# nlesc-dirac/sagecal

Measured on NVIDIA H100. Metric: baseline_visibilities_per_sec_predict_jacobian, higher is better.
Workload: dtype f64

## Files before the change

### sagecal_b200/csrc/internal.cuh

```cuda
#pragma once
#include <cuda_runtime.h>
#include <stdint.h>
#include <stdio.h>
#include <stdlib.h>

#define DB_CHECK(call)                                                                          \
  do {                                                                                          \
    cudaError_t err__ = (call);                                                                 \
    if (err__ != cudaSuccess) {                                                                 \
      fprintf(stderr, "dirac_b200: CUDA error %s at %s:%d: %s\n", cudaGetErrorName(err__),      \
              __FILE__, __LINE__, cudaGetErrorString(err__));                                   \
      exit(1);          \
    }                                                                                           \
  } while (0)


#define TILE_P 8
#define TILE_Q 32
#define TILE_THREADS (TILE_P * TILE_Q)

struct TileDesc {
  short pb, qb;
};

// ... 229 lines not shown

struct GramArgs {
  const double2 *coh;
  const unsigned char *flag;
  const TileDesc *tiles;
  double *T;
  long long R;
  int N, Nbase;
  int k0;
  int t_begin, t_end, t_step;
};

struct AssembleArgs {
  const double *T;
  const double *pblk;
  double *JTJ;
  double *Hst;
  const TileDesc *tiles;
  const short2 *blpq;
  int N, Nbase;
};

struct BatchAssembleArgs {
  const double *T;
  const double *pp;
  const int *list;
  const int *tix;
  const int *poff;
  double *JTJ;
  double *Hst;
  const TileDesc *tiles;
  const short2 *blpq;
  int N, Nbase;
};

enum { DB_OPT_CP_ROWS = 0, DB_OPT_LINE_DIRECT = 1, DB_OPT_OS_CONSISTENT = 2,
       DB_OPT_RTR_NU_UNJOINED = 3, DB_OPT_ADMM_LM = 4, DB_OPT_COUNT = 8 };
int db_opt(int id);
int db_sm_count();
static inline int db_cp_max_slices(int Nbase, int tilesz) {
  const int nbg = (Nbase + 255) / 256;
  int nsl = (db_sm_count() + nbg - 1) / nbg;
  if ((tilesz + 31) / 32 > nsl) nsl = (tilesz + 31) / 32;
  return nsl;
}

extern "C" {
void db_launch_coh_to_planar(const double2 *src, double2 *dst, long long r0, int nr, int M,
                             long long R, cudaStream_t st);
void db_launch_coh_from_planar(const double2 *src, double2 *dst, long long r0, int nr, int M,
                               long long R, cudaStream_t st);
void db_launch_vis_to_planar(const double2 *src, double2 *dst, long long R, cudaStream_t st);
void db_launch_vis_from_planar(const double2 *src, double2 *dst, long long R, cudaStream_t st);
void db_launch_grad_tma(const GradArgs *a, int ntile, cudaStream_t st);
void db_launch_grad_window_tma(const GradArgs *a, int ntile, long long r_lo, long long r_hi,
                               cudaStream_t st);
void db_launch_grad_band_tma(const GradArgs *a, int ntile, int nchan, cudaStream_t st);
int db_cluster_pass_nblocks(int ntile, int nt, int tslice);
void db_launch_cluster_pass(const ClusterPassArgs *a, int ntile, cudaStream_t st);
int db_cluster_pass_forms_hidden(int N, int Nbase);
void db_launch_coh_gram(const GramArgs *a, int ntile, int nk, cudaStream_t st);
void db_launch_assemble(const AssembleArgs *a, int ntile, cudaStream_t st);
void db_launch_copy_add_diag(const double *A0, double *A, int n, double mu, cudaStream_t st);
int db_chol_max_n();
int db_chol_available();
size_t db_chol_ws_doubles(int n);
int db_tri_available(int n);
void db_chol_set_step(const double *pcur, double *pnew, double *sc, double *zero);
void db_launch_tri_solve(const double *L, int n, const double *b, double *x, cudaStream_t st);
void db_launch_tri_solve_ld(const double *L, int ld, int n, const double *b, double *x,
                            cudaStream_t st);
void db_launch_chol_factor_batched(const double *A, int n, const double *mu, double *ws,
                                   long long ws_stride, int *info, int nb, cudaStream_t st);
void db_launch_chol_solve(const double *A, int n, double mu, const double *b, double *x, double *ws,
                          int *info, cudaStream_t st);
int db_bigtri_available(int n);
size_t db_bigtri_ws_doubles(int n);
// ... 13 lines not shown
```

### sagecal_b200/csrc/kernels_lm.cu

```cuda
#include "internal.cuh"

struct Gram {
  double d[4];
  double2 o[6];
  __device__ __forceinline__ double2 at(int u, int v) const {
    if (u == v) return make_double2(d[u], 0.0);
    int lo = u < v ? u : v, hi = u < v ? v : u;
    int idx = (lo == 0) ? (hi - 1) : (lo == 1 ? (hi + 1) : 5);
    double2 z = o[idx];
    return (u < v) ? z : make_double2(z.x, -z.y);
  }
};


__device__ __forceinline__ void assemble_baseline(const AssembleArgs &a, int p, int q, long long b,
                                                  int sub) {
  Gram G;
  {
    const double2 *Tb = reinterpret_cast<const double2 *>(a.T + b * 16);
    double2 t0 = Tb[0], t1 = Tb[1];
    G.d[0] = t0.x; G.d[1] = t0.y; G.d[2] = t1.x; G.d[3] = t1.y;
#pragma unroll
    for (int z = 0; z < 6; z++) G.o[z] = Tb[2 + z];
  }
  double2 Jp[4], Jq[4];
  load_jones(a.pblk, p, Jp);
  load_jones(a.pblk, q, Jq);
  const int ld = 8 * a.N;
#pragma unroll
  for (int i = 0; i < 2; i++)
#pragma unroll
    for (int l = 0; l < 2; l++)
#pragma unroll
      for (int j = 0; j < 2; j++)
#pragma unroll
        for (int lp = 0; lp < 2; lp++) {
          double2 z = make_double2(0.0, 0.0);
#pragma unroll
          for (int aa = 0; aa < 2; aa++)
#pragma unroll
            for (int bb = 0; bb < 2; bb++) {
              double2 jj = cmul(Jq[2 * j + aa], Jp[2 * i + bb]);
              cfma(z, jj, G.at(2 * l + aa, 2 * bb + lp));
            }
          if (sub != ((i * 2 + l) * 2 + j) * 2 + lp) continue;
          const int r0 = 8 * p + 2 * (2 * i + l);
          const int c0 = 8 * q + 2 * (2 * j + lp);
          a.JTJ[(long long)r0 * ld + c0] = z.x;
          a.JTJ[(long long)r0 * ld + c0 + 1] = z.y;
          a.JTJ[(long long)(r0 + 1) * ld + c0] = z.y;
          a.JTJ[(long long)(r0 + 1) * ld + c0 + 1] = -z.x;
          a.JTJ[(long long)c0 * ld + r0] = z.x;
          a.JTJ[(long long)(c0 + 1) * ld + r0] = z.y;
          a.JTJ[(long long)c0 * ld + r0 + 1] = z.y;
          a.JTJ[(long long)(c0 + 1) * ld + r0 + 1] = -z.x;
        }
  double2 Qq[4], Qp[4];
  mat_ahb(Jq, Jq, Qq);
  mat_ahb(Jp, Jp, Qp);
  double2 Hp[4], Hq[4];
#pragma unroll
  for (int l = 0; l < 2; l++)
#pragma unroll
    for (int lp = 0; lp < 2; lp++) {
      double2 hp = make_double2(0.0, 0.0), hq = make_double2(0.0, 0.0);
#pragma unroll
      for (int aa = 0; aa < 2; aa++)
#pragma unroll
        for (int bb = 0; bb < 2; bb++) {
          cfma(hp, Qq[2 * aa + bb], G.at(2 * lp + bb, 2 * l + aa));
          cfma(hq, Qp[2 * aa + bb], G.at(2 * aa + l, 2 * bb + lp));
        }
      Hp[2 * l + lp] = hp;
      Hq[2 * l + lp] = hq;
    }
  if (sub == 0) atomicAdd(a.Hst + 4 * p + 0, Hp[0].x);
  if (sub == 1) atomicAdd(a.Hst + 4 * p + 1, Hp[3].x);
  if (sub == 2) atomicAdd(a.Hst + 4 * p + 2, Hp[1].x);
  if (sub == 3) atomicAdd(a.Hst + 4 * p + 3, Hp[1].y);
  if (sub == 4) atomicAdd(a.Hst + 4 * q + 0, Hq[0].x);
  if (sub == 5) atomicAdd(a.Hst + 4 * q + 1, Hq[3].x);
  if (sub == 6) atomicAdd(a.Hst + 4 * q + 2, Hq[1].x);
  if (sub == 7) atomicAdd(a.Hst + 4 * q + 3, Hq[1].y);
}

__device__ __forceinline__ void assemble_lin(const AssembleArgs &a) {
  const long long gid = (long long)blockIdx.x * blockDim.x + threadIdx.x;
  const long long b = gid >> 4;
  if (b >= a.Nbase) return;
  const short2 pq = a.blpq[b];
  assemble_baseline(a, pq.x, pq.y, b, (int)(gid & 15));
}

__global__ void __launch_bounds__(256)
k_assemble_offdiag(AssembleArgs a) {
  assemble_lin(a);
}

__global__ void __launch_bounds__(256)
k_assemble_offdiag_batched(BatchAssembleArgs b) {
  const int k = b.list[blockIdx.y];
  AssembleArgs a;
  a.T = b.T + (long long)b.tix[k] * b.Nbase * 16;
  a.pblk = b.pp + b.poff[k];
  a.JTJ = b.JTJ + (long long)blockIdx.y * 64 * b.N * b.N;
  a.Hst = b.Hst + (long long)blockIdx.y * 4 * b.N;
  a.tiles = b.tiles;
  a.blpq = b.blpq;
  a.N = b.N;
  a.Nbase = b.Nbase;
  assemble_lin(a);
}

__device__ __forceinline__ void assemble_diag_station(const double *__restrict__ Hst,
                                                      double *__restrict__ JTJ, int N, int s);

__global__ void k_assemble_diag(const double *__restrict__ Hst, double *__restrict__ JTJ, int N) {
  int s = blockIdx.x * blockDim.x + threadIdx.x;
  if (s >= N) return;
  assemble_diag_station(Hst, JTJ, N, s);
}
__global__ void k_assemble_diag_batched(const double *__restrict__ Hst, double *__restrict__ JTJ,
                                        int N) {
  int s = blockIdx.x * blockDim.x + threadIdx.x;
  if (s >= N) return;
  assemble_diag_station(Hst + (long long)blockIdx.y * 4 * N, JTJ + (long long)blockIdx.y * 64 * N * N,
                        N, s);
}
__device__ __forceinline__ void assemble_diag_station(const double *__restrict__ Hst,
                                                      double *__restrict__ JTJ, int N, int s) {
  const double h00 = Hst[4 * s], h11 = Hst[4 * s + 1], hr = Hst[4 * s + 2], hi = Hst[4 * s + 3];
  const int ld = 8 * N;
  for (int i = 0; i < 2; i++) {
    double blk[4][4] = {{h00, 0.0, hr, hi}, {0.0, h00, -hi, hr}, {hr, -hi, h11, 0.0},
                        {hi, hr, 0.0, h11}};
    for (int r = 0; r < 8; r++)
      for (int c = 0; c < 8; c++) {
        double v = 0.0;
        if ((r >> 2) == i && (c >> 2) == i) v = blk[r & 3][c & 3];
        if ((r >> 2) == i) JTJ[(long long)(8 * s + r) * ld + 8 * s + c] = v;
      }
  }
}

__global__ void __launch_bounds__(128)
k_batch_mu0(const double *__restrict__ Hst, double *__restrict__ mu, int N, double tau) {
  __shared__ double sv[4];
  const double *H = Hst + (long long)blockIdx.x * 4 * N;
  double mx = 0.0;
  for (int s = threadIdx.x; s < N; s += blockDim.x) {
    const double a = H[4 * s], b = H[4 * s + 1];
    if (fabs(a) > fabs(mx)) mx = a;
    if (fabs(b) > fabs(mx)) mx = b;
  }
#pragma unroll
  for (int o = 16; o > 0; o >>= 1) {
    const double other = __shfl_xor_sync(0xffffffffu, mx, o);
    if (fabs(other) > fabs(mx)) mx = other;
  }
  if ((threadIdx.x & 31) == 0) sv[threadIdx.x >> 5] = mx;
  __syncthreads();
  if (threadIdx.x == 0) {
    for (int i = 1; i < 4; i++)
      if (fabs(sv[i]) > fabs(mx)) mx = sv[i];
    mu[blockIdx.x] = tau * mx;
  }
}

__global__ void k_batch_add_diag(const double *__restrict__ A0, double *__restrict__ A,
                                 const double *__restrict__ mu, int n) {
  const long long nn = (long long)n * n;
  const long long i = (long long)blockIdx.x * blockDim.x + threadIdx.x;
  if (i < nn) {
    double v = A0[(long long)blockIdx.y * nn + i];
    if (i / n == i % n) v += mu[blockIdx.y];
    A[(long long)blockIdx.y * nn + i] = v;
  }
}

__global__ void k_copy_add_diag(const double *__restrict__ A0, double *__restrict__ A, int n,
                                double mu) {
  long long i = (long long)blockIdx.x * blockDim.x + threadIdx.x;
  long long nn = (long long)n * n;
  if (i < nn) {
    double v = A0[i];
    if (i / n == i % n) v += mu;
    A[i] = v;
  }
}

__global__ void k_extract_diag(const double *__restrict__ A, double *__restrict__ dst, int n) {
// ... 39 lines not shown
  if (i < n) g[i] = g[i] - 0.5 * y[i] - 0.5 * rho * (p[i] - bz[i]);
}

extern "C" {
void db_launch_lm_aug_rhs(double *jte, const double *p, const double *y, const double *bz,
                          double rho, int n, cudaStream_t st) {
  k_lm_aug_rhs<<<(n + 255) / 256, 256, 0, st>>>(jte, p, y, bz, rho, n);
}
void db_launch_lm_step(const double *p, const double *Dp, const double *jte, double *pnew,
                       double *sc, double *zero, int n, cudaStream_t st) {
  k_lm_step<<<1, 512, 0, st>>>(p, Dp, jte, pnew, sc, zero, n);
}
void db_launch_extract_diag(const double *A, double *dst, int n, cudaStream_t st) {
  k_extract_diag<<<(n + 127) / 128, 128, 0, st>>>(A, dst, n);
}
void db_launch_assemble(const AssembleArgs *a, int ntile, cudaStream_t st) {
  (void)ntile;
  k_assemble_offdiag<<<(a->Nbase * 16 + 255) / 256, 256, 0, st>>>(*a);
  k_assemble_diag<<<(a->N + 63) / 64, 64, 0, st>>>(a->Hst, a->JTJ, a->N);
}
void db_launch_assemble_batched(const BatchAssembleArgs *b, int ntile, int nb, double tau,
                                double *mu, double *Afac, cudaStream_t st) {
  (void)ntile;
  dim3 g1((b->Nbase * 16 + 255) / 256, nb);
  k_assemble_offdiag_batched<<<g1, 256, 0, st>>>(*b);
  dim3 g2((b->N + 63) / 64, nb);
  k_assemble_diag_batched<<<g2, 64, 0, st>>>(b->Hst, b->JTJ, b->N);
  k_batch_mu0<<<nb, 128, 0, st>>>(b->Hst, mu, b->N, tau);
  if (!Afac) return;
  const int n = 8 * b->N;
  const long long nn = (long long)n * n;
  dim3 g3((unsigned)((nn + 255) / 256), nb);
  k_batch_add_diag<<<g3, 256, 0, st>>>(b->JTJ, Afac, mu, n);
}
void db_launch_copy_add_diag(const double *A0, double *A, int n, double mu, cudaStream_t st) {
  long long nn = (long long)n * n;
  k_copy_add_diag<<<(unsigned)((nn + 255) / 256), 256, 0, st>>>(A0, A, n, mu);
}
}
```

### sagecal_b200/csrc/lm.cu

```cuda
#include <float.h>
#include <math.h>
#include <string.h>
#include <vector>

#include "../../include/dirac_b200.h"
#include "problem.h"

#define CS_CHECK(call)                                                                     \
  do {                                                                                     \
    cusolverStatus_t s__ = (call);                                                         \
    if (s__ != CUSOLVER_STATUS_SUCCESS) {                                                  \
      fprintf(stderr, "dirac_b200: cuSOLVER error %d at %s:%d\n", (int)s__, __FILE__, __LINE__); \
      exit(1);                                                                             \
    }                                                                                      \
  } while (0)
#define CB_CHECK(call)                                                                     \
  do {                                                                                     \
    cublasStatus_t s__ = (call);                                                           \
    if (s__ != CUBLAS_STATUS_SUCCESS) {                                                    \
      fprintf(stderr, "dirac_b200: cuBLAS error %d at %s:%d\n", (int)s__, __FILE__, __LINE__); \
      exit(1);                                                                             \
    }                                                                                      \
  } while (0)

extern "C" {
void db_launch_weighted_jtj(const WeightedJtjArgs *a, int ntile, cudaStream_t st);
void db_launch_sum_abs(const double2 *v, long long R, long long r0, long long r1, double *partials,
                       double *out, unsigned int *counter, cudaStream_t st);
void db_launch_update_weights(const double2 *e, double2 *wt, long long R, long long r0,
                              long long r1, double nu0, double *partials, double *out,
                              unsigned int *counter, cudaStream_t st);
void db_launch_scale_vis(double2 *v, long long R, long long r0, long long r1, double alpha,
                         int set_const, cudaStream_t st);
void db_launch_extract_diag(const double *A, double *dst, int n, cudaStream_t st);
void db_launch_assemble_batched(const BatchAssembleArgs *b, int ntile, int nb, double tau,
                                double *mu, double *Afac, cudaStream_t st);
void db_launch_lm_step(const double *p, const double *Dp, const double *jte, double *pnew,
                       double *sc, double *zero, int n, cudaStream_t st);
void db_launch_os_shift(const double2 *e, const double2 *wt, double2 *eps, double2 *wout, long long R,
                        long long row_sub0, long long nrow_sub, long long row_chunk0, long long kl,
                        long long nJ, cudaStream_t st);
}

template <typename T>
static T *dalloc(size_t n) {
  return (T *)db_malloc(n * sizeof(T) + 16);
}

void db_lm_init(dirac_b200_problem *pr) {
  LMWork &w = pr->lm;
  if (w.ready) return;
// ... 7 lines not shown
  w.JTJ = dalloc<double>((size_t)n8 * n8);
  w.JTe = d.scal + 64 + n8;
  w.JTe_new = d.scal + 64 + 2 * n8;
  w.Hst = dalloc<double>((size_t)4 * d.N);
  w.Dp = d.scal + 64;
  w.pnew = dalloc<double>(n8);
  w.plast = dalloc<double>(n8);
  w.pold = dalloc<double>(n8);
  w.devinfo = reinterpret_cast<int *>(d.scal + 64 + 3 * n8);
  w.tau = dalloc<double>(n8);
  w.svdS = w.svdU = w.svdVT = nullptr;
  w.wbuf = w.ebuf = nullptr;
  w.os_eps = w.os_w = nullptr;
  w.HP = w.HQ = nullptr;
  w.JB = w.LB = nullptr;
  w.pref_slot = (int *)malloc(sizeof(int) * d.M);
  for (int k = 0; k < d.M; k++) w.pref_slot[k] = -1;
  w.jtj0_cur = nullptr;
  w.jtj_spec = nullptr;
  {
    const int nbg = (d.Nbase + 255) / 256;
    const int nsl = db_cp_max_slices(d.Nbase, d.tilesz);
    w.jte_part = dalloc<double>((size_t)nbg * (nsl + 1) * n8);
  }
  DB_CHECK(cudaEventCreateWithFlags(&w.ev_mail, cudaEventDisableTiming));
  DB_CHECK(cudaMallocHost((void **)&w.h_vec, sizeof(double) * (5 * n8 + 4 * d.N + 64)));
  static cusolverDnHandle_t g_cs = nullptr;
  static cublasHandle_t g_cb = nullptr;
  if (!g_cs) {
    CS_CHECK(cusolverDnCreate(&g_cs));
// ... 43 lines not shown
  if (w.os_eps) return;
  w.os_eps = dalloc<double2>((size_t)4 * pr->d.R);
  w.os_w = dalloc<double2>((size_t)4 * pr->d.R);
}

void db_lm_free(dirac_b200_problem *pr) {
  LMWork &w = pr->lm;
  if (!w.ready) return;
  db_free(w.T); db_free(w.Tsub); db_free(w.JTJ0); db_free(w.JTJ);
  db_free(w.Hst); db_free(w.pnew); db_free(w.plast); db_free(w.pold); db_free(w.jte_part);
  db_free(w.tau); db_free(w.cswork); db_free(w.dbuf);
  if (w.bt_ws) db_free(w.bt_ws);
  if (w.svdS) { db_free(w.svdS); db_free(w.svdU); db_free(w.svdVT); }
  if (w.wbuf) { db_free(w.wbuf); db_free(w.ebuf); db_free(w.HP); db_free(w.HQ); }
  if (w.os_eps) { db_free(w.os_eps); db_free(w.os_w); }
  if (w.JB) {
    db_free(w.JB); db_free(w.LB); db_free(w.HB); db_free(w.mu_dev); db_free(w.binfo_dev);
    db_free(w.LBptr_dev); db_free(w.blist_dev); db_free(w.btix_dev); db_free(w.bpoff_dev);
    cudaFreeHost(w.h_mu); cudaFreeHost(w.h_binfo);
  }
  free(w.pref_slot);
  cudaEventDestroy(w.ev_mail);
  cudaFreeHost(w.h_vec);
  free(w.T_valid);
  w.ready = false;
}

static int pick_tslice(const DevProblem &d, int nt) {
  int target_ctas = db_sm_count();
  int slices = (target_ctas + d.ntile - 1) / d.ntile;
  if (slices < 1) slices = 1;
  int ts = (nt + slices - 1) / slices;
// ... 39 lines not shown
  db_count_launch(1);
}

static void gram(dirac_b200_problem *pr, int k, int t0, int t1, int step, double *Tdst) {
  DevProblem &d = pr->d;
  GramArgs a;
  a.coh = d.coh; a.flag = d.flag; a.tiles = d.tiles; a.T = Tdst; a.R = d.R; a.N = d.N;
  a.Nbase = d.Nbase; a.k0 = k; a.t_begin = t0; a.t_end = t1; a.t_step = step;
  db_prof_begin(3, (double)((t1 - t0 + step - 1) / step) * d.Nbase * 65.0 + 128.0 * d.Nbase,
                d.stream);
  db_launch_coh_gram(&a, d.ntile, 1, d.stream);
  db_prof_end(d.stream);
  db_count_launch(1);
}

static void assemble(dirac_b200_problem *pr, const double *T, const double *pblk_dev,
                     double *JTJ) {
  DevProblem &d = pr->d;
  LMWork &w = pr->lm;
  DB_CHECK(cudaMemsetAsync(w.Hst, 0, sizeof(double) * 4 * d.N, d.stream));
  AssembleArgs a;
  a.T = T; a.pblk = pblk_dev; a.JTJ = JTJ; a.Hst = w.Hst; a.tiles = d.tiles; a.blpq = d.blpq;
  a.N = d.N;
  a.Nbase = d.Nbase;
  db_prof_begin(4, 128.0 * d.Nbase + 8.0 * 64.0 * d.N * d.N, d.stream);
  db_launch_assemble(&a, d.ntile, d.stream);
  db_prof_end(d.stream);
  db_count_launch(2);
}

static void weighted_jtj(dirac_b200_problem *pr, int k, int t0, int t1, const double *pblk_dev,
                         const double2 *wt, double *JTJ) {
  DevProblem &d = pr->d;
  LMWork &w = pr->lm;
  const int n = w.n8;
  DB_CHECK(cudaMemsetAsync(JTJ, 0, sizeof(double) * (size_t)n * n, d.stream));
  DB_CHECK(cudaMemsetAsync(w.HP, 0, sizeof(double) * 20 * d.N, d.stream));
  DB_CHECK(cudaMemsetAsync(w.HQ, 0, sizeof(double) * 20 * d.N, d.stream));
  if (t1 <= t0) return;
  WeightedJtjArgs a;
  a.coh_k = d.coh + (size_t)k * 4 * d.R;
  a.wt = wt; a.flag = d.flag; a.pblk = pblk_dev; a.tiles = d.tiles; a.JTJ = JTJ; a.HP = w.HP;
  a.HQ = w.HQ; a.R = d.R; a.N = d.N; a.Nbase = d.Nbase; a.t_begin = t0; a.t_end = t1;
// ... 22 lines not shown
static int enqueue_solve(dirac_b200_problem *pr, double mu, int linsolv, double eps1) {
  DevProblem &d = pr->d;
  LMWork &w = pr->lm;
  const int n = w.n8;
  int *hinfo = (int *)(w.h_vec + 4 * n + 4 * d.N);
  hinfo[0] = hinfo[1] = 0;
  if (linsolv == 0 && w.own_chol) {
    db_prof_begin(5, 0.0, d.stream);
    db_launch_chol_solve(w.jtj0_cur ? w.jtj0_cur : w.JTJ0, n, mu, w.JTe, w.Dp, w.cswork, w.devinfo,
                         d.stream);
    db_prof_end(d.stream);
    db_count_launch(1);
    w.step_fused = w.step_armed;
    return 1;
  }
  db_launch_copy_add_diag(w.jtj0_cur ? w.jtj0_cur : w.JTJ0, w.JTJ, n, mu, d.stream);
  db_count_launch(1);
  DB_CHECK(cudaMemcpyAsync(w.Dp, w.JTe, sizeof(double) * n, cudaMemcpyDeviceToDevice, d.stream));
  db_prof_begin(5, 0.0, d.stream);
  if (linsolv == 0) {
    CS_CHECK(cusolverDnDpotrf(w.cs, CUBLAS_FILL_MODE_LOWER, n, w.JTJ, n, w.cswork, w.lwork,
                              w.devinfo));
    if (w.bt_ws) {
      DB_CHECK(cudaMemsetAsync(w.devinfo + 1, 0, sizeof(int), d.stream));
      db_launch_bigtri_solve(w.JTJ, n, n, w.JTe, w.Dp, w.bt_ws, ++w.bt_epoch, 1, d.stream);
      db_count_launch(4);
    } else {
      CS_CHECK(cusolverDnDpotrs(w.cs, CUBLAS_FILL_MODE_LOWER, n, 1, w.JTJ, n, w.Dp, n,
                                w.devinfo + 1));
      db_count_launch(2);
    }
  } else if (linsolv == 1) {
// ... 37 lines not shown
  return 1;
}

static double nrm2sq(const double *v, int n) {
  double s = 0.0;
  for (int i = 0; i < n; i++) s += v[i] * v[i];
  return s;
}

void db_prefactor_sweep(dirac_b200_problem *pr, double tau) {
  DevProblem &d = pr->d;
  db_lm_init(pr);
  LMWork &w = pr->lm;
  const int n = w.n8;
  const size_t nn = (size_t)n * n;
  if ((double)d.M * nn * 16.0 > 24e9) return;
  const bool own_batch = w.own_chol && db_tri_available(n) && !getenv("DIRAC_B200_BATCH_CUSOLVER");
  const size_t lstride = own_batch ? db_chol_ws_doubles(n) : nn;
  w.lb_stride = lstride;
  w.lb_ld = own_batch ? 32 * ((n + 31) / 32) : n;
  if (!w.JB) {
    w.JB = dalloc<double>(nn * d.M);
    w.LB = dalloc<double>(lstride * d.M);
    w.HB = dalloc<double>((size_t)4 * d.N * d.M);
    w.mu_dev = dalloc<double>(d.M);
    w.binfo_dev = dalloc<int>(2 * d.M);
    w.LBptr_dev = (double **)dalloc<double *>(d.M);
    w.blist_dev = dalloc<int>(d.M);
    w.btix_dev = dalloc<int>(d.M);
    w.bpoff_dev = dalloc<int>(d.M);
    DB_CHECK(cudaMallocHost((void **)&w.h_mu, sizeof(double) * d.M));
    DB_CHECK(cudaMallocHost((void **)&w.h_binfo, sizeof(int) * 2 * d.M));
    std::vector<int> tix(d.M), poff(d.M);
    std::vector<double *> ptr(d.M);
    for (int k = 0; k < d.M; k++) {
      tix[k] = d.h_clus[k].chunk0;
      poff[k] = d.h_chunk_poff[d.h_clus[k].chunk0];
// ... 24 lines not shown
    db_prof_end(d.stream);
    db_count_launch(1);
    for (int kk = k; kk < k1; kk++) w.T_valid[d.h_clus[kk].chunk0] = 1;
    k = k1;
  }
  for (int k = 0; k < d.M; k++) {
    w.pref_slot[k] = -1;
    if (d.h_clus[k].nchunk != 1) continue;
    w.pref_slot[k] = (int)list.size();
    list.push_back(k);
  }
  const int nb = (int)list.size();
  if (nb == 0) return;
  DB_CHECK(cudaMemcpyAsync(w.blist_dev, list.data(), sizeof(int) * nb, cudaMemcpyHostToDevice,
                           d.stream));
  DB_CHECK(cudaMemsetAsync(w.HB, 0, sizeof(double) * 4 * d.N * nb, d.stream));
  BatchAssembleArgs b;
  b.T = w.T; b.pp = d.pp; b.list = w.blist_dev; b.tix = w.btix_dev; b.poff = w.bpoff_dev;
  b.JTJ = w.JB; b.Hst = w.HB; b.tiles = d.tiles; b.blpq = d.blpq; b.N = d.N; b.Nbase = d.Nbase;
  db_prof_begin(4, nb * (128.0 * d.Nbase + 8.0 * 64.0 * d.N * d.N), d.stream);
  db_launch_assemble_batched(&b, d.ntile, nb, tau, w.mu_dev, own_batch ? nullptr : w.LB, d.stream);
  db_prof_end(d.stream);
  db_count_launch(4);
  db_prof_begin(5, 0.0, d.stream);
  if (own_batch) {
    db_launch_chol_factor_batched(w.JB, n, w.mu_dev, w.LB, (long long)lstride, w.binfo_dev, nb,
                                  d.stream);
    db_count_launch(1);
  } else if (n <= 1024) {
    CS_CHECK(cusolverDnDpotrfBatched(w.cs, CUBLAS_FILL_MODE_LOWER, n, w.LBptr_dev, n, w.binfo_dev, nb));
    db_count_launch(1);
  } else {
    enum { NS = 4 };
    static cudaStream_t fs[NS];
    static cusolverDnHandle_t fh[NS];
    static double *fwork[NS];
    static int flwork = 0;
    static cudaEvent_t fev[NS], fstart;
// ... 230 lines not shown
      break;
    }
    if (os && randomize) {
      subI.resize(Nsubsets);
      for (int i = 0; i < Nsubsets; ++i) {
        const int j = rand() % (i + 1);
        subI[i] = subI[j];
        subI[j] = i;
      }
    }
    for (int ositer = 0; ositer < max_os_iter; ositer++) {
      double mx = 0.0;
      const int slot = (!wt && !os && kiter == 0 && linsolv == 0) ? w.pref_slot[k] : -1;
      const bool prefac = slot >= 0;
      const bool need_mx = (kiter == 0) && !prefac;
      w.jtj0_cur = prefac ? w.JB + (size_t)slot * n * n : nullptr;
      if (os) {
        const int l = randomize ? subI[ositer] : (os_shift + kiter + ositer) % Nsubsets;
        os_subset_system(pr, k, t0, t1, l, pblk_dev, wt);
        DB_CHECK(cudaMemcpyAsync(hjte, w.JTe, sizeof(double) * n, cudaMemcpyDeviceToHost,
                                 d.stream));
      } else if (prefac) {
        w.pref_slot[k] = -1;
      } else if (wt) {
        weighted_jtj(pr, k, t0, t1, pblk_dev, wt, w.JTJ0);
      } else if (w.jtj_spec) {
        w.jtj0_cur = w.jtj_spec;
        w.jtj_spec = nullptr;
      } else {
        assemble(pr, Tfull, pblk_dev, w.JTJ0);
      }
      if (need_mx) {
        if (wt || os_misaligned) {
          db_launch_extract_diag(w.JTJ0, w.JTe_new, n, d.stream);
          db_count_launch(1);
          DB_CHECK(cudaMemcpyAsync(hsc, w.JTe_new, sizeof(double) * n, cudaMemcpyDeviceToHost,
                                   d.stream));
        } else {
          DB_CHECK(cudaMemcpyAsync(hH, w.Hst, sizeof(double) * 4 * d.N, cudaMemcpyDeviceToHost,
                                   d.stream));
        }
      }
      if (need_mx || os) db_stream_sync(d.stream);
      if (need_mx) {
        if (wt || os_misaligned) {
// ... 410 lines not shown
  int t0, t1;
  chunk_range(d, clus, chunk, &t0, &t1);
  db_upload_vis(pr, xd, w.dbuf);
  db_upload_vis(pr, wt, w.wbuf);
  DB_CHECK(cudaMemcpyAsync(w.pnew, pblk, sizeof(double) * n, cudaMemcpyHostToDevice, d.stream));
  db_cluster_pass(pr, clus, w.pnew, w.dbuf, nullptr, 1, 0, w.JTe, 1, t0, t1, w.wbuf);
  weighted_jtj(pr, clus, t0, t1, w.pnew, w.wbuf, w.JTJ0);
  double c = db_read_scalar(pr, 1);
  if (JTe) DB_CHECK(cudaMemcpy(JTe, w.JTe, sizeof(double) * n, cudaMemcpyDeviceToHost));
  if (JTJ)
    DB_CHECK(cudaMemcpy(JTJ, w.JTJ0, sizeof(double) * (size_t)n * n, cudaMemcpyDeviceToHost));
  DB_CHECK(cudaGetLastError());
  return c;
}

extern "C" void dirac_b200_os_normal_eq(dirac_b200_problem *pr, int clus, int chunk, int l,
                                        const double *pblk, const double *xd, const double *wt,
                                        double *JTJ, double *JTe, long long *path) {
  DevProblem &d = pr->d;
  db_lm_init(pr);
  robust_init(pr);
  LMWork &w = pr->lm;
  const int n = w.n8;
  int t0, t1;
  chunk_range(d, clus, chunk, &t0, &t1);
  db_upload_vis(pr, xd, w.dbuf);
  if (wt) db_upload_vis(pr, wt, w.wbuf);
  DB_CHECK(cudaMemcpyAsync(w.pnew, pblk, sizeof(double) * n, cudaMemcpyHostToDevice, d.stream));
  const OsPath p = os_subset_system(pr, clus, t0, t1, l, w.pnew, wt ? w.wbuf : nullptr);
  DB_CHECK(cudaMemcpyAsync(JTe, w.JTe, sizeof(double) * n, cudaMemcpyDeviceToHost, d.stream));
// ... 110 lines not shown
```

### sagecal_b200/csrc/problem.h

```cpp
#pragma once
#include <cusolverDn.h>
#include <cublas_v2.h>

#include <vector>

#include "../../include/dirac_b200.h"
#include "internal.cuh"

struct LMWork {
  bool ready;
  int n8;
  double *T;
  unsigned char *T_valid;
  double *Tsub;
  double *JTJ0, *JTJ;
  double *JTe, *JTe_new;
  double *Hst;
  double *Dp;
  double *pnew;
  double *h_vec;
  int *devinfo;
  double *cswork;
  int lwork;
  bool own_chol;
// ... 13 lines not shown
  double2 *os_eps, *os_w;
  double *HP, *HQ;
  double *plast;
  double *pold;
  double *JB, *LB;
  size_t lb_stride;
  int lb_ld, binfo_step;
  double *HB;
  double *mu_dev;
  double *h_mu;
  int *binfo_dev, *h_binfo;
  double **LBptr_dev;
  int *blist_dev, *btix_dev, *bpoff_dev;
  int *pref_slot;
  const double *jtj0_cur;
};

struct dirac_b200_problem {
  DevProblem d;
  double *partials;
  int npartials;
  double2 *res;
  double2 *vis_stage;
  double *g;
  LMWork lm;
  int own_stream;
  int rank, world;
  void (*allreduce)(void *dev, long long count, void *stream, void *user);
  void *comm_user;
  int m_global;
// ... 119 lines not shown
```

Measured before the change: 6.222 billion.

## Restructure LM normal-equation assembly into station-sum and tiled damped-assembly kernels

Replaces the per-baseline JTJ assembly, which used atomics for the station Hessian diagonals and a separate diagonal kernel, with two kernels. One computes per-station sums with warp reductions and no atomics. The other writes JTJ tiles with vectorized stores, adding the damping mu directly and optionally writing only the lower triangle. This removes the memset, the copy_add_diag pass and the batched add-diag pass, and can drop the JB buffer when it is not needed. The cost is recomputing the tiles for each damping trial when assembling in place. The measured workload is predict/jacobian visibilities, which may not exercise this LM path.

```diff
diff --git a/sagecal_b200/csrc/internal.cuh b/sagecal_b200/csrc/internal.cuh
--- a/sagecal_b200/csrc/internal.cuh
+++ b/sagecal_b200/csrc/internal.cuh
@@ -267,23 +267,15 @@
 struct AssembleArgs {
   const double *T;
   const double *pblk;
-  double *JTJ;
-  double *Hst;
-  const TileDesc *tiles;
-  const short2 *blpq;
-  int N, Nbase;
-};
-
-struct BatchAssembleArgs {
-  const double *T;
-  const double *pp;
   const int *list;
   const int *tix;
   const int *poff;
   double *JTJ;
+  long long stride;
   double *Hst;
-  const TileDesc *tiles;
-  const short2 *blpq;
+  const double *mu_dev;
+  double mu;
+  int lower;
   int N, Nbase;
 };
 
@@ -313,7 +305,9 @@
 void db_launch_cluster_pass(const ClusterPassArgs *a, int ntile, cudaStream_t st);
 int db_cluster_pass_forms_hidden(int N, int Nbase);
 void db_launch_coh_gram(const GramArgs *a, int ntile, int nk, cudaStream_t st);
-void db_launch_assemble(const AssembleArgs *a, int ntile, cudaStream_t st);
+void db_launch_station_sums(const AssembleArgs *a, int nb, cudaStream_t st);
+void db_launch_assemble_tiles(const AssembleArgs *a, int nb, cudaStream_t st);
+void db_launch_batch_mu0(const double *Hst, double *mu, int N, double tau, int nb, cudaStream_t st);
 void db_launch_copy_add_diag(const double *A0, double *A, int n, double mu, cudaStream_t st);
 int db_chol_max_n();
 int db_chol_available();
diff --git a/sagecal_b200/csrc/kernels_lm.cu b/sagecal_b200/csrc/kernels_lm.cu
--- a/sagecal_b200/csrc/kernels_lm.cu
+++ b/sagecal_b200/csrc/kernels_lm.cu
@@ -13,133 +13,144 @@
 };
 
 
-__device__ __forceinline__ void assemble_baseline(const AssembleArgs &a, int p, int q, long long b,
-                                                  int sub) {
+__device__ __forceinline__ long long pair_baseline(int p, int q, int N) {
+  return (long long)p * (2 * N - p - 1) / 2 + (q - p - 1);
+}
+
+__device__ __forceinline__ Gram load_gram(const double *T, long long b) {
   Gram G;
-  {
-    const double2 *Tb = reinterpret_cast<const double2 *>(a.T + b * 16);
-    double2 t0 = Tb[0], t1 = Tb[1];
-    G.d[0] = t0.x; G.d[1] = t0.y; G.d[2] = t1.x; G.d[3] = t1.y;
-#pragma unroll
-    for (int z = 0; z < 6; z++) G.o[z] = Tb[2 + z];
-  }
-  double2 Jp[4], Jq[4];
-  load_jones(a.pblk, p, Jp);
-  load_jones(a.pblk, q, Jq);
-  const int ld = 8 * a.N;
-#pragma unroll
-  for (int i = 0; i < 2; i++)
+  const double2 *Tb = reinterpret_cast<const double2 *>(T + b * 16);
+  const double2 t0 = __ldg(Tb), t1 = __ldg(Tb + 1);
+  G.d[0] = t0.x; G.d[1] = t0.y; G.d[2] = t1.x; G.d[3] = t1.y;
+#pragma unroll
+  for (int z = 0; z < 6; z++) G.o[z] = __ldg(Tb + 2 + z);
+  return G;
+}
+
+struct AsmSys {
+  const double *T, *J;
+  double *A, *H;
+  double mu;
+};
+__device__ __forceinline__ AsmSys asm_sys(const AssembleArgs &a, int y) {
+  AsmSys s;
+  if (a.list) {
+    const int k = a.list[y];
+    s.T = a.T + (long long)a.tix[k] * a.Nbase * 16;
+    s.J = a.pblk + a.poff[k];
+  } else {
+    s.T = a.T;
+    s.J = a.pblk;
+  }
+  s.A = a.JTJ + (long long)y * a.stride;
+  s.H = a.Hst + (long long)y * 4 * a.N;
+  s.mu = a.mu_dev ? a.mu_dev[y] : a.mu;
+  return s;
+}
+
+__global__ void __launch_bounds__(256)
+k_station_sums(AssembleArgs a) {
+  const AsmSys S = asm_sys(a, blockIdx.y);
+  const int s = blockIdx.x * 8 + (threadIdx.x >> 5);
+  const int lane = threadIdx.x & 31;
+  if (s >= a.N) return;
+  double h0 = 0.0, h1 = 0.0, h2 = 0.0, h3 = 0.0;
+  for (int o = lane; o < a.N; o += 32) {
+    if (o == s) continue;
+    const bool sp = s < o;
+    const Gram G = load_gram(S.T, sp ? pair_baseline(s, o, a.N) : pair_baseline(o, s, a.N));
+    double2 Jo[4], Qo[4];
+    load_jones(S.J, o, Jo);
+    mat_ahb(Jo, Jo, Qo);
+    double2 h[4];
 #pragma unroll
     for (int l = 0; l < 2; l++)
 #pragma unroll
-      for (int j = 0; j < 2; j++)
-#pragma unroll
-        for (int lp = 0; lp < 2; lp++) {
-          double2 z = make_double2(0.0, 0.0);
-#pragma unroll
-          for (int aa = 0; aa < 2; aa++)
-#pragma unroll
-            for (int bb = 0; bb < 2; bb++) {
-              double2 jj = cmul(Jq[2 * j + aa], Jp[2 * i + bb]);
-              cfma(z, jj, G.at(2 * l + aa, 2 * bb + lp));
-            }
-          if (sub != ((i * 2 + l) * 2 + j) * 2 + lp) continue;
-          const int r0 = 8 * p + 2 * (2 * i + l);
-          const int c0 = 8 * q + 2 * (2 * j + lp);
-          a.JTJ[(long long)r0 * ld + c0] = z.x;
-          a.JTJ[(long long)r0 * ld + c0 + 1] = z.y;
-          a.JTJ[(long long)(r0 + 1) * ld + c0] = z.y;
-          a.JTJ[(long long)(r0 + 1) * ld + c0 + 1] = -z.x;
-          a.JTJ[(long long)c0 * ld + r0] = z.x;
-          a.JTJ[(long long)(c0 + 1) * ld + r0] = z.y;
-          a.JTJ[(long long)c0 * ld + r0 + 1] = z.y;
-          a.JTJ[(long long)(c0 + 1) * ld + r0 + 1] = -z.x;
+      for (int lp = 0; lp < 2; lp++) {
+        double2 z = make_double2(0.0, 0.0);
+#pragma unroll
+        for (int aa = 0; aa < 2; aa++)
+#pragma unroll
+          for (int bb = 0; bb < 2; bb++)
+            cfma(z, Qo[2 * aa + bb], sp ? G.at(2 * lp + bb, 2 * l + aa) : G.at(2 * aa + l, 2 * bb + lp));
+        h[2 * l + lp] = z;
+      }
+    h0 += h[0].x;
+    h1 += h[3].x;
+    h2 += h[1].x;
+    h3 += h[1].y;
+  }
+  h0 = warp_sum(h0);
+  h1 = warp_sum(h1);
+  h2 = warp_sum(h2);
+  h3 = warp_sum(h3);
+  if (lane == 0) {
+    S.H[4 * s] = h0;
+    S.H[4 * s + 1] = h1;
+    S.H[4 * s + 2] = h2;
+    S.H[4 * s + 3] = h3;
+  }
+}
+
+__global__ void __launch_bounds__(256)
+k_assemble_tiles(AssembleArgs a) {
+  const int P = blockIdx.x;
+  const int qcta = blockIdx.y * 64;
+  if (a.lower && qcta + 64 <= P) return;
+  const int warp = threadIdx.x >> 5, lane = threadIdx.x & 31;
+  const int q0 = qcta + 8 * warp;
+  if (q0 >= a.N || (a.lower && q0 + 8 <= P)) return;
+  const AsmSys S = asm_sys(a, blockIdx.z);
+  const int Q = q0 + (lane >> 2);
+  const int jl = lane & 3, j = jl >> 1, lp = jl & 1;
+  const long long ld = 8ll * a.N;
+  if (Q == P) {
+    const double h00 = S.H[4 * P], h11 = S.H[4 * P + 1], hr = S.H[4 * P + 2], hi = S.H[4 * P + 3];
+    const double blk[4][4] = {{h00, 0.0, hr, hi}, {0.0, h00, -hi, hr}, {hr, -hi, h11, 0.0},
+                              {hi, hr, 0.0, h11}};
+#pragma unroll
+    for (int il = 0; il < 4; il++) {
+      const int i = il >> 1, l = il & 1;
+      double2 v0 = make_double2(0.0, 0.0), v1 = v0;
+      if (i == j) {
+        const double m = (l == lp) ? S.mu : 0.0;
+        v0 = lp ? make_double2(blk[2 * l][2], blk[2 * l][3]) : make_double2(blk[2 * l][0], blk[2 * l][1]);
+        v1 = lp ? make_double2(blk[2 * l + 1][2], blk[2 * l + 1][3])
+                : make_double2(blk[2 * l + 1][0], blk[2 * l + 1][1]);
+        v0.x += m;
+        v1.y += m;
+      }
+      const long long r0 = 8ll * P + 2 * il;
+      *reinterpret_cast<double2 *>(S.A + r0 * ld + 8ll * Q + 2 * jl) = v0;
+      *reinterpret_cast<double2 *>(S.A + (r0 + 1) * ld + 8ll * Q + 2 * jl) = v1;
+    }
+    return;
+  }
+  if (Q < a.N) {
+    const bool pq = P < Q;
+    const Gram G = load_gram(S.T, pq ? pair_baseline(P, Q, a.N) : pair_baseline(Q, P, a.N));
+    double2 JP[4], JQ[4];
+    load_jones(S.J, P, JP);
+    load_jones(S.J, Q, JQ);
+    const double2 Jj[2] = {j ? JQ[2] : JQ[0], j ? JQ[3] : JQ[1]};
+#pragma unroll
+    for (int il = 0; il < 4; il++) {
+      const int i = il >> 1, l = il & 1;
+      double2 z = make_double2(0.0, 0.0);
+#pragma unroll
+      for (int aa = 0; aa < 2; aa++)
+#pragma unroll
+        for (int bb = 0; bb < 2; bb++) {
+          if (pq)
+            cfma(z, cmul(Jj[aa], JP[2 * i + bb]),
+                 lp ? G.at(2 * l + aa, 2 * bb + 1) : G.at(2 * l + aa, 2 * bb));
+          else
+            cfma(z, cmul(JP[2 * i + aa], Jj[bb]), lp ? G.at(2 + aa, 2 * bb + l) : G.at(aa, 2 * bb + l));
         }
-  double2 Qq[4], Qp[4];
-  mat_ahb(Jq, Jq, Qq);
-  mat_ahb(Jp, Jp, Qp);
-  double2 Hp[4], Hq[4];
-#pragma unroll
-  for (int l = 0; l < 2; l++)
-#pragma unroll
-    for (int lp = 0; lp < 2; lp++) {
-      double2 hp = make_double2(0.0, 0.0), hq = make_double2(0.0, 0.0);
-#pragma unroll
-      for (int aa = 0; aa < 2; aa++)
-#pragma unroll
-        for (int bb = 0; bb < 2; bb++) {
-          cfma(hp, Qq[2 * aa + bb], G.at(2 * lp + bb, 2 * l + aa));
-          cfma(hq, Qp[2 * aa + bb], G.at(2 * aa + l, 2 * bb + lp));
-        }
-      Hp[2 * l + lp] = hp;
-      Hq[2 * l + lp] = hq;
+      const long long r0 = 8ll * P + 2 * il;
+      *reinterpret_cast<double2 *>(S.A + r0 * ld + 8ll * Q + 2 * jl) = z;
+      *reinterpret_cast<double2 *>(S.A + (r0 + 1) * ld + 8ll * Q + 2 * jl) = make_double2(z.y, -z.x);
     }
-  if (sub == 0) atomicAdd(a.Hst + 4 * p + 0, Hp[0].x);
-  if (sub == 1) atomicAdd(a.Hst + 4 * p + 1, Hp[3].x);
-  if (sub == 2) atomicAdd(a.Hst + 4 * p + 2, Hp[1].x);
-  if (sub == 3) atomicAdd(a.Hst + 4 * p + 3, Hp[1].y);
-  if (sub == 4) atomicAdd(a.Hst + 4 * q + 0, Hq[0].x);
-  if (sub == 5) atomicAdd(a.Hst + 4 * q + 1, Hq[3].x);
-  if (sub == 6) atomicAdd(a.Hst + 4 * q + 2, Hq[1].x);
-  if (sub == 7) atomicAdd(a.Hst + 4 * q + 3, Hq[1].y);
-}
-
-__device__ __forceinline__ void assemble_lin(const AssembleArgs &a) {
-  const long long gid = (long long)blockIdx.x * blockDim.x + threadIdx.x;
-  const long long b = gid >> 4;
-  if (b >= a.Nbase) return;
-  const short2 pq = a.blpq[b];
-  assemble_baseline(a, pq.x, pq.y, b, (int)(gid & 15));
-}
-
-__global__ void __launch_bounds__(256)
-k_assemble_offdiag(AssembleArgs a) {
-  assemble_lin(a);
-}
-
-__global__ void __launch_bounds__(256)
-k_assemble_offdiag_batched(BatchAssembleArgs b) {
-  const int k = b.list[blockIdx.y];
-  AssembleArgs a;
-  a.T = b.T + (long long)b.tix[k] * b.Nbase * 16;
-  a.pblk = b.pp + b.poff[k];
-  a.JTJ = b.JTJ + (long long)blockIdx.y * 64 * b.N * b.N;
-  a.Hst = b.Hst + (long long)blockIdx.y * 4 * b.N;
-  a.tiles = b.tiles;
-  a.blpq = b.blpq;
-  a.N = b.N;
-  a.Nbase = b.Nbase;
-  assemble_lin(a);
-}
-
-__device__ __forceinline__ void assemble_diag_station(const double *__restrict__ Hst,
-                                                      double *__restrict__ JTJ, int N, int s);
-
-__global__ void k_assemble_diag(const double *__restrict__ Hst, double *__restrict__ JTJ, int N) {
-  int s = blockIdx.x * blockDim.x + threadIdx.x;
-  if (s >= N) return;
-  assemble_diag_station(Hst, JTJ, N, s);
-}
-__global__ void k_assemble_diag_batched(const double *__restrict__ Hst, double *__restrict__ JTJ,
-                                        int N) {
-  int s = blockIdx.x * blockDim.x + threadIdx.x;
-  if (s >= N) return;
-  assemble_diag_station(Hst + (long long)blockIdx.y * 4 * N, JTJ + (long long)blockIdx.y * 64 * N * N,
-                        N, s);
-}
-__device__ __forceinline__ void assemble_diag_station(const double *__restrict__ Hst,
-                                                      double *__restrict__ JTJ, int N, int s) {
-  const double h00 = Hst[4 * s], h11 = Hst[4 * s + 1], hr = Hst[4 * s + 2], hi = Hst[4 * s + 3];
-  const int ld = 8 * N;
-  for (int i = 0; i < 2; i++) {
-    double blk[4][4] = {{h00, 0.0, hr, hi}, {0.0, h00, -hi, hr}, {hr, -hi, h11, 0.0},
-                        {hi, hr, 0.0, h11}};
-    for (int r = 0; r < 8; r++)
-      for (int c = 0; c < 8; c++) {
-        double v = 0.0;
-        if ((r >> 2) == i && (c >> 2) == i) v = blk[r & 3][c & 3];
-        if ((r >> 2) == i) JTJ[(long long)(8 * s + r) * ld + 8 * s + c] = v;
-      }
   }
 }
 
@@ -164,17 +175,6 @@
     for (int i = 1; i < 4; i++)
       if (fabs(sv[i]) > fabs(mx)) mx = sv[i];
     mu[blockIdx.x] = tau * mx;
-  }
-}
-
-__global__ void k_batch_add_diag(const double *__restrict__ A0, double *__restrict__ A,
-                                 const double *__restrict__ mu, int n) {
-  const long long nn = (long long)n * n;
-  const long long i = (long long)blockIdx.x * blockDim.x + threadIdx.x;
-  if (i < nn) {
-    double v = A0[(long long)blockIdx.y * nn + i];
-    if (i / n == i % n) v += mu[blockIdx.y];
-    A[(long long)blockIdx.y * nn + i] = v;
   }
 }
 
@@ -244,24 +244,14 @@
 void db_launch_extract_diag(const double *A, double *dst, int n, cudaStream_t st) {
   k_extract_diag<<<(n + 127) / 128, 128, 0, st>>>(A, dst, n);
 }
-void db_launch_assemble(const AssembleArgs *a, int ntile, cudaStream_t st) {
-  (void)ntile;
-  k_assemble_offdiag<<<(a->Nbase * 16 + 255) / 256, 256, 0, st>>>(*a);
-  k_assemble_diag<<<(a->N + 63) / 64, 64, 0, st>>>(a->Hst, a->JTJ, a->N);
-}
-void db_launch_assemble_batched(const BatchAssembleArgs *b, int ntile, int nb, double tau,
-                                double *mu, double *Afac, cudaStream_t st) {
-  (void)ntile;
-  dim3 g1((b->Nbase * 16 + 255) / 256, nb);
-  k_assemble_offdiag_batched<<<g1, 256, 0, st>>>(*b);
-  dim3 g2((b->N + 63) / 64, nb);
-  k_assemble_diag_batched<<<g2, 64, 0, st>>>(b->Hst, b->JTJ, b->N);
-  k_batch_mu0<<<nb, 128, 0, st>>>(b->Hst, mu, b->N, tau);
-  if (!Afac) return;
-  const int n = 8 * b->N;
-  const long long nn = (long long)n * n;
-  dim3 g3((unsigned)((nn + 255) / 256), nb);
-  k_batch_add_diag<<<g3, 256, 0, st>>>(b->JTJ, Afac, mu, n);
+void db_launch_station_sums(const AssembleArgs *a, int nb, cudaStream_t st) {
+  k_station_sums<<<dim3((a->N + 7) / 8, nb), 256, 0, st>>>(*a);
+}
+void db_launch_assemble_tiles(const AssembleArgs *a, int nb, cudaStream_t st) {
+  k_assemble_tiles<<<dim3(a->N, (a->N + 63) / 64, nb), 256, 0, st>>>(*a);
+}
+void db_launch_batch_mu0(const double *Hst, double *mu, int N, double tau, int nb, cudaStream_t st) {
+  k_batch_mu0<<<nb, 128, 0, st>>>(Hst, mu, N, tau);
 }
 void db_launch_copy_add_diag(const double *A0, double *A, int n, double mu, cudaStream_t st) {
   long long nn = (long long)n * n;
diff --git a/sagecal_b200/csrc/lm.cu b/sagecal_b200/csrc/lm.cu
--- a/sagecal_b200/csrc/lm.cu
+++ b/sagecal_b200/csrc/lm.cu
@@ -33,8 +33,6 @@
 void db_launch_scale_vis(double2 *v, long long R, long long r0, long long r1, double alpha,
                          int set_const, cudaStream_t st);
 void db_launch_extract_diag(const double *A, double *dst, int n, cudaStream_t st);
-void db_launch_assemble_batched(const BatchAssembleArgs *b, int ntile, int nb, double tau,
-                                double *mu, double *Afac, cudaStream_t st);
 void db_launch_lm_step(const double *p, const double *Dp, const double *jte, double *pnew,
                        double *sc, double *zero, int n, cudaStream_t st);
 void db_launch_os_shift(const double2 *e, const double2 *wt, double2 *eps, double2 *wout, long long R,
@@ -72,6 +70,7 @@
   w.os_eps = w.os_w = nullptr;
   w.HP = w.HQ = nullptr;
   w.JB = w.LB = nullptr;
+  w.sys_T = w.sys_p = w.sys_H = nullptr;
   w.pref_slot = (int *)malloc(sizeof(int) * d.M);
   for (int k = 0; k < d.M; k++) w.pref_slot[k] = -1;
   w.jtj0_cur = nullptr;
@@ -145,8 +144,9 @@
   if (w.svdS) { db_free(w.svdS); db_free(w.svdU); db_free(w.svdVT); }
   if (w.wbuf) { db_free(w.wbuf); db_free(w.ebuf); db_free(w.HP); db_free(w.HQ); }
   if (w.os_eps) { db_free(w.os_eps); db_free(w.os_w); }
-  if (w.JB) {
-    db_free(w.JB); db_free(w.LB); db_free(w.HB); db_free(w.mu_dev); db_free(w.binfo_dev);
+  if (w.LB) {
+    if (w.JB) db_free(w.JB);
+    db_free(w.LB); db_free(w.HB); db_free(w.mu_dev); db_free(w.binfo_dev);
     db_free(w.LBptr_dev); db_free(w.blist_dev); db_free(w.btix_dev); db_free(w.bpoff_dev);
     cudaFreeHost(w.h_mu); cudaFreeHost(w.h_binfo);
   }
@@ -216,19 +216,39 @@
   db_count_launch(1);
 }
 
+static AssembleArgs assemble_args(const DevProblem &d, const double *T, const double *pblk_dev,
+                                  double *Hst) {
+  AssembleArgs a;
+  memset(&a, 0, sizeof(a));
+  a.T = T; a.pblk = pblk_dev; a.Hst = Hst; a.N = d.N; a.Nbase = d.Nbase;
+  return a;
+}
+
+static void station_sums(dirac_b200_problem *pr, const AssembleArgs &a, int nb) {
+  DevProblem &d = pr->d;
+  db_prof_begin(4, nb * 256.0 * d.Nbase, d.stream);
+  db_launch_station_sums(&a, nb, d.stream);
+  db_prof_end(d.stream);
+  db_count_launch(1);
+}
+
+static void assemble_tiles(dirac_b200_problem *pr, const AssembleArgs &a, int nb) {
+  DevProblem &d = pr->d;
+  const double n = 8.0 * d.N;
+  db_prof_begin(4, nb * (a.lower ? 128.0 * d.Nbase + 4.0 * n * (n + 1) : 256.0 * d.Nbase + 8.0 * n * n),
+                d.stream);
+  db_launch_assemble_tiles(&a, nb, d.stream);
+  db_prof_end(d.stream);
+  db_count_launch(1);
+}
+
 static void assemble(dirac_b200_problem *pr, const double *T, const double *pblk_dev,
                      double *JTJ) {
-  DevProblem &d = pr->d;
-  LMWork &w = pr->lm;
-  DB_CHECK(cudaMemsetAsync(w.Hst, 0, sizeof(double) * 4 * d.N, d.stream));
-  AssembleArgs a;
-  a.T = T; a.pblk = pblk_dev; a.JTJ = JTJ; a.Hst = w.Hst; a.tiles = d.tiles; a.blpq = d.blpq;
-  a.N = d.N;
-  a.Nbase = d.Nbase;
-  db_prof_begin(4, 128.0 * d.Nbase + 8.0 * 64.0 * d.N * d.N, d.stream);
-  db_launch_assemble(&a, d.ntile, d.stream);
-  db_prof_end(d.stream);
-  db_count_launch(2);
+  AssembleArgs a = assemble_args(pr->d, T, pblk_dev, pr->lm.Hst);
+  station_sums(pr, a, 1);
+  if (!JTJ) return;
+  a.JTJ = JTJ;
+  assemble_tiles(pr, a, 1);
 }
 
 static void weighted_jtj(dirac_b200_problem *pr, int k, int t0, int t1, const double *pblk_dev,
@@ -281,8 +301,18 @@
     w.step_fused = w.step_armed;
     return 1;
   }
-  db_launch_copy_add_diag(w.jtj0_cur ? w.jtj0_cur : w.JTJ0, w.JTJ, n, mu, d.stream);
-  db_count_launch(1);
+  if (linsolv == 0 && w.sys_T) {
+    AssembleArgs a = assemble_args(d, w.sys_T, w.sys_p, const_cast<double *>(w.sys_H));
+    a.JTJ = w.JTJ;
+    a.mu = mu;
+    a.lower = 1;
+    assemble_tiles(pr, a, 1);
+  } else {
+    db_prof_begin(4, 16.0 * n * n, d.stream);
+    db_launch_copy_add_diag(w.jtj0_cur ? w.jtj0_cur : w.JTJ0, w.JTJ, n, mu, d.stream);
+    db_prof_end(d.stream);
+    db_count_launch(1);
+  }
   DB_CHECK(cudaMemcpyAsync(w.Dp, w.JTe, sizeof(double) * n, cudaMemcpyDeviceToDevice, d.stream));
   db_prof_begin(5, 0.0, d.stream);
   if (linsolv == 0) {
@@ -350,13 +380,14 @@
   LMWork &w = pr->lm;
   const int n = w.n8;
   const size_t nn = (size_t)n * n;
-  if ((double)d.M * nn * 16.0 > 24e9) return;
   const bool own_batch = w.own_chol && db_tri_available(n) && !getenv("DIRAC_B200_BATCH_CUSOLVER");
+  const bool keep_jb = w.own_chol;
+  if ((double)d.M * nn * 8.0 * (keep_jb ? 2 : 1) > 24e9) return;
   const size_t lstride = own_batch ? db_chol_ws_doubles(n) : nn;
   w.lb_stride = lstride;
   w.lb_ld = own_batch ? 32 * ((n + 31) / 32) : n;
-  if (!w.JB) {
-    w.JB = dalloc<double>(nn * d.M);
+  if (!w.LB) {
+    w.JB = keep_jb ? dalloc<double>(nn * d.M) : nullptr;
     w.LB = dalloc<double>(lstride * d.M);
     w.HB = dalloc<double>((size_t)4 * d.N * d.M);
     w.mu_dev = dalloc<double>(d.M);
@@ -411,14 +442,23 @@
   if (nb == 0) return;
   DB_CHECK(cudaMemcpyAsync(w.blist_dev, list.data(), sizeof(int) * nb, cudaMemcpyHostToDevice,
                            d.stream));
-  DB_CHECK(cudaMemsetAsync(w.HB, 0, sizeof(double) * 4 * d.N * nb, d.stream));
-  BatchAssembleArgs b;
-  b.T = w.T; b.pp = d.pp; b.list = w.blist_dev; b.tix = w.btix_dev; b.poff = w.bpoff_dev;
-  b.JTJ = w.JB; b.Hst = w.HB; b.tiles = d.tiles; b.blpq = d.blpq; b.N = d.N; b.Nbase = d.Nbase;
-  db_prof_begin(4, nb * (128.0 * d.Nbase + 8.0 * 64.0 * d.N * d.N), d.stream);
-  db_launch_assemble_batched(&b, d.ntile, nb, tau, w.mu_dev, own_batch ? nullptr : w.LB, d.stream);
-  db_prof_end(d.stream);
-  db_count_launch(4);
+  AssembleArgs b = assemble_args(d, w.T, d.pp, w.HB);
+  b.list = w.blist_dev; b.tix = w.btix_dev; b.poff = w.bpoff_dev;
+  station_sums(pr, b, nb);
+  db_launch_batch_mu0(w.HB, w.mu_dev, d.N, tau, nb, d.stream);
+  db_count_launch(1);
+  if (keep_jb) {
+    b.JTJ = w.JB;
+    b.stride = (long long)nn;
+    assemble_tiles(pr, b, nb);
+  }
+  if (!own_batch) {
+    b.JTJ = w.LB;
+    b.stride = (long long)lstride;
+    b.mu_dev = w.mu_dev;
+    b.lower = 1;
+    assemble_tiles(pr, b, nb);
+  }
   db_prof_begin(5, 0.0, d.stream);
   if (own_batch) {
     db_launch_chol_factor_batched(w.JB, n, w.mu_dev, w.LB, (long long)lstride, w.binfo_dev, nb,
@@ -679,7 +719,11 @@
       const int slot = (!wt && !os && kiter == 0 && linsolv == 0) ? w.pref_slot[k] : -1;
       const bool prefac = slot >= 0;
       const bool need_mx = (kiter == 0) && !prefac;
-      w.jtj0_cur = prefac ? w.JB + (size_t)slot * n * n : nullptr;
+      w.jtj0_cur = (prefac && w.JB) ? w.JB + (size_t)slot * n * n : nullptr;
+      const bool in_place = !w.own_chol && linsolv == 0 && !wt && !os;
+      w.sys_T = in_place ? Tfull : nullptr;
+      w.sys_p = pblk_dev;
+      w.sys_H = prefac ? w.HB + (size_t)slot * 4 * d.N : w.Hst;
       if (os) {
         const int l = randomize ? subI[ositer] : (os_shift + kiter + ositer) % Nsubsets;
         os_subset_system(pr, k, t0, t1, l, pblk_dev, wt);
@@ -693,7 +737,7 @@
         w.jtj0_cur = w.jtj_spec;
         w.jtj_spec = nullptr;
       } else {
-        assemble(pr, Tfull, pblk_dev, w.JTJ0);
+        assemble(pr, Tfull, pblk_dev, in_place ? nullptr : w.JTJ0);
       }
       if (need_mx) {
         if (wt || os_misaligned) {
@@ -1134,6 +1178,79 @@
   return c;
 }
 
+extern "C" void dirac_b200_assemble_damped(dirac_b200_problem *pr, int clus, int chunk,
+                                           const double *pblk, int nmu, const double *mus,
+                                           int factor, double *out, int *info) {
+  DevProblem &d = pr->d;
+  db_lm_init(pr);
+  LMWork &w = pr->lm;
+  const int n = w.n8;
+  int t0, t1;
+  chunk_range(d, clus, chunk, &t0, &t1);
+  DB_CHECK(cudaMemcpyAsync(w.pnew, pblk, sizeof(double) * n, cudaMemcpyHostToDevice, d.stream));
+  gram(pr, clus, t0, t1, 1, w.Tsub);
+  assemble(pr, w.Tsub, w.pnew, nullptr);
+  for (int i = 0; i < nmu; i++) {
+    AssembleArgs a = assemble_args(d, w.Tsub, w.pnew, w.Hst);
+    a.JTJ = w.JTJ;
+    a.mu = mus[i];
+    a.lower = 1;
+    assemble_tiles(pr, a, 1);
+    if (factor)
+      CS_CHECK(cusolverDnDpotrf(w.cs, CUBLAS_FILL_MODE_LOWER, n, w.JTJ, n, w.cswork, w.lwork,
+                                w.devinfo));
+    DB_CHECK(cudaMemcpyAsync(out + (size_t)i * n * n, w.JTJ, sizeof(double) * (size_t)n * n,
+                             cudaMemcpyDeviceToHost, d.stream));
+    if (factor)
+      DB_CHECK(cudaMemcpyAsync(info + i, w.devinfo, sizeof(int), cudaMemcpyDeviceToHost, d.stream));
+    db_stream_sync(d.stream);
+  }
+  DB_CHECK(cudaGetLastError());
+}
+
+extern "C" void dirac_b200_assemble_batch(dirac_b200_problem *pr, const double *pp, const int *list,
+                                          int nb, double tau, int lower, double *mu_out, double *out) {
+  DevProblem &d = pr->d;
+  db_lm_init(pr);
+  DB_CHECK(cudaMemcpy(d.pp, pp, sizeof(double) * d.npar, cudaMemcpyHostToDevice));
+  LMWork &w = pr->lm;
+  const size_t nn = (size_t)w.n8 * w.n8;
+  std::vector<int> tix(d.M), poff(d.M);
+  for (int k = 0; k < d.M; k++) {
+    tix[k] = d.h_clus[k].chunk0;
+    poff[k] = d.h_chunk_poff[tix[k]];
+  }
+  for (int y = 0; y < nb; y++) {
+    const int k = list[y];
+    int t0, t1;
+    chunk_range(d, k, 0, &t0, &t1);
+    gram(pr, k, t0, t1, 1, w.T + (size_t)tix[k] * d.Nbase * 16);
+    w.T_valid[tix[k]] = 1;
+  }
+  int *ibuf = dalloc<int>(nb + 2 * d.M);
+  double *H = dalloc<double>((size_t)4 * d.N * nb), *mu = dalloc<double>(nb);
+  double *A = dalloc<double>(nn * nb);
+  DB_CHECK(cudaMemcpy(ibuf, list, sizeof(int) * nb, cudaMemcpyHostToDevice));
+  DB_CHECK(cudaMemcpy(ibuf + nb, tix.data(), sizeof(int) * d.M, cudaMemcpyHostToDevice));
+  DB_CHECK(cudaMemcpy(ibuf + nb + d.M, poff.data(), sizeof(int) * d.M, cudaMemcpyHostToDevice));
+  AssembleArgs b = assemble_args(d, w.T, d.pp, H);
+  b.list = ibuf; b.tix = ibuf + nb; b.poff = ibuf + nb + d.M;
+  b.JTJ = A;
+  b.stride = (long long)nn;
+  station_sums(pr, b, nb);
+  db_launch_batch_mu0(H, mu, d.N, tau, nb, d.stream);
+  if (lower) {
+    b.mu_dev = mu;
+    b.lower = 1;
+  }
+  assemble_tiles(pr, b, nb);
+  DB_CHECK(cudaMemcpyAsync(mu_out, mu, sizeof(double) * nb, cudaMemcpyDeviceToHost, d.stream));
+  DB_CHECK(cudaMemcpyAsync(out, A, sizeof(double) * nn * nb, cudaMemcpyDeviceToHost, d.stream));
+  db_stream_sync(d.stream);
+  db_free(ibuf); db_free(H); db_free(mu); db_free(A);
+  DB_CHECK(cudaGetLastError());
+}
+
 extern "C" void dirac_b200_os_normal_eq(dirac_b200_problem *pr, int clus, int chunk, int l,
                                         const double *pblk, const double *xd, const double *wt,
                                         double *JTJ, double *JTe, long long *path) {
diff --git a/sagecal_b200/csrc/problem.h b/sagecal_b200/csrc/problem.h
--- a/sagecal_b200/csrc/problem.h
+++ b/sagecal_b200/csrc/problem.h
@@ -51,6 +51,7 @@
   int *blist_dev, *btix_dev, *bpoff_dev;
   int *pref_slot;
   const double *jtj0_cur;
+  const double *sys_T, *sys_p, *sys_H;
 };
 
 struct dirac_b200_problem {
```

After: 6.668 billion (median of 6 runs). 1.07x the previous value.
